# facebookresearch/fast3r

Measured on AMD Instinct MI355X. Metric: views/sec (512^2, ViT-L) single forward pass at N=320, higher is better.
Workload: dtype fp16

## Files before the change

fast3r_amd/csrc/f3r_capi.hip:

```cpp
#include <stdarg.h>
#include <stdio.h>

#include "f3r_common.h"

namespace {
thread_local char g_err[512] = "";
}

void f3r_set_error(const char* fmt, ...) {
  va_list ap;
  va_start(ap, fmt);
  vsnprintf(g_err, sizeof(g_err), fmt, ap);
  va_end(ap);
}

int f3r_check_launch(const char* what) {
  hipError_t e = hipGetLastError();
  if (e != hipSuccess) {
    f3r_set_error("%s: launch failed: %s", what, hipGetErrorString(e));
    return F3R_ERR_LAUNCH;
  }
  return F3R_OK;
}

extern "C" int f3r_version(void) { return 380;  }

extern "C" int f3r_wall_clock_khz(void) {
  int dev = 0, khz = 0;
  if (hipGetDevice(&dev) != hipSuccess || hipDeviceGetAttribute(&khz, hipDeviceAttributeWallClockRate, dev) != hipSuccess) {
    (void)hipGetLastError();
    return 0;
  }
  return khz;
}

extern "C" const char* f3r_last_error_string(void) { return g_err; }

extern "C" size_t f3r_sizeof(int what) {
  switch (what) {
    case 0: return sizeof(f3r_gemm_args);
// ... 26 lines not shown
```

fast3r_amd/csrc/f3r_gemm.hip:

```cpp
#include <stdlib.h>

#include "f3r_common.h"
#include "f3r_gemm_epi.h"

namespace {

constexpr int BM = 128, BN = 128, BK = 64, NT = 256;
constexpr int TILE_ELEMS = 128 * 64;
constexpr int GEMM_LDS_BYTES = 2 * 2 * TILE_ELEMS * 2;

__device__ __forceinline__ int swz(int row, int chunk) { return row * 64 + ((chunk ^ ((row >> 1) & 7)) << 3); }

struct ConvRow {
  int b, oy, ox;
  bool ok;
};

template <class T, int A_MODE, int EPI, int GLDS>
__global__ __launch_bounds__(NT, 2) void gemm_kernel(const f3r_gemm_args p) {
  extern __shared__ __attribute__((aligned(16))) uint16_t smem[];
  uint16_t* As = smem;
  uint16_t* Ws = smem + 2 * TILE_ELEMS;

  const int tid = threadIdx.x;
// ... 284 lines not shown
    }
    if (!f3r_gemm_asm_f8_eligible(a, &why)) {
      f3r_set_error("f3r_gemm: split W2F8 (fp8 low plane) but the launch is not eligible for the hand-scheduled kernel: %s", why);
      return F3R_ERR_UNSUPPORTED;
    }
    return f3r_gemm_asm_f8_launch(a, (hipStream_t)stream);
  }
  F3R_REQUIRE(a.epi == F3R_EPI_GENERIC || (!a.out_f8 && !a.out_relu_f8 && !a.fin_w), "f3r_gemm: out_f8 / out_relu_f8 / fin_w need the generic epilogue (epi %d)", a.epi);
  const int planes = a.split ? 2 : 1;
  F3R_REQUIRE(a.Kpad > 0 && a.Kpad % (64 * planes) == 0, "f3r_gemm: Kpad %d must be a positive multiple of %d", a.Kpad, 64 * planes);
  const int Kpad1 = a.Kpad / planes;
  F3R_REQUIRE((a.split != F3R_SPLIT_X3 && a.split != F3R_SPLIT_X3F8) || (a.A_lo && al16(a.A_lo) && !a.a_relu), "f3r_gemm: X3 / X3F8 split needs A_lo (16-byte aligned) and no a_relu");
  if (a.split == F3R_SPLIT_X3F8)
    F3R_REQUIRE(a.a_mode == F3R_A_CONV3X3 && a.dtype == F3R_F16 && a.conv_C % 128 == 0 && a.w_scale && (((uintptr_t)a.w_scale) & 3) == 0,
                "f3r_gemm: X3F8 needs a 3x3 convolution with conv_C %% 128 == 0 (got %d), fp16 planes and w_scale", a.conv_C);
  F3R_REQUIRE((a.kernel_sel >= 0 && a.kernel_sel <= 7) || a.kernel_sel == 9 || a.kernel_sel >= 16, "f3r_gemm: bad kernel_sel %d", a.kernel_sel);
  F3R_REQUIRE(a.N % 4 == 0, "f3r_gemm: N %d must be a multiple of 4", a.N);
  F3R_REQUIRE(al16(a.A) && al16(a.W), "f3r_gemm: A/W must be 16-byte aligned");
  F3R_REQUIRE(a.dtype == F3R_F16 || a.dtype == F3R_BF16, "f3r_gemm: bad dtype %d", a.dtype);
  if (a.a_mode == F3R_A_PLAIN) {
    F3R_REQUIRE(a.K > 0 && a.K % 8 == 0 && a.K <= Kpad1, "f3r_gemm: K %d must be a multiple of 8 and <= Kpad", a.K);
    F3R_REQUIRE(a.lda % 8 == 0 && a.lda >= a.K, "f3r_gemm: lda %lld must be a multiple of 8 and >= K", (long long)a.lda);
  } else if (a.a_mode == F3R_A_CONV3X3) {
    F3R_REQUIRE(a.conv_C > 0 && a.conv_C % 8 == 0, "f3r_gemm: conv_C %d must be a multiple of 8", a.conv_C);
    F3R_REQUIRE(Kpad1 == 9 * ((a.conv_C + 63) / 64) * 64, "f3r_gemm: conv Kpad %d != 9*roundup(C,64) per plane", a.Kpad);
    F3R_REQUIRE(a.epi == F3R_EPI_GENERIC, "f3r_gemm: conv3x3 supports only the generic epilogue");
    F3R_REQUIRE(a.conv_stride == 1 || a.conv_stride == 2, "f3r_gemm: conv stride %d", a.conv_stride);
    F3R_REQUIRE(a.conv_OH == (a.conv_H + 2 - 3) / a.conv_stride + 1 && a.conv_OW == (a.conv_W + 2 - 3) / a.conv_stride + 1,
                "f3r_gemm: conv output dims inconsistent");
    F3R_REQUIRE(a.conv_OH > 0 && a.conv_OW > 0 && a.M % ((int64_t)a.conv_OH * a.conv_OW) == 0, "f3r_gemm: conv M not a multiple of OH*OW");
  } else {
// ... 69 lines not shown
```

fast3r_amd/csrc/f3r_gemm256.hip:

```cpp
#include "f3r_gemm256_impl.h"

int f3r_gemm256_run_bf16(const f3r_gemm_args& a, hipStream_t stream, int stagger);
int f3r_gemm256_run_conv_f8_fin(const f3r_gemm_args& a, hipStream_t stream);

bool f3r_gemm256_eligible(const f3r_gemm_args& a) {
  if (a.N % 128 != 0) return false;
  if (a.epi == F3R_EPI_QKV) {
    const int Dq = a.qkv_dq ? a.qkv_dq : a.N / 3;
    if (Dq % 256 != 0 || ((a.N - Dq) / 2) % 256 != 0) return false;
  }
  const int Kpad1 = a.split ? a.Kpad / 2 : a.Kpad;
  if (Kpad1 % 64 != 0) return false;
  if (a.a_mode == F3R_A_PLAIN) {
    if (a.K != Kpad1) return false;
    if ((int64_t)256 * a.lda * 2 >= (1ll << 32)) return false;
  } else {
    if (a.a_relu || a.conv_C % 64 != 0) return false;
    if (a.M / ((int64_t)a.conv_OH * a.conv_OW) * a.conv_H * a.conv_W * a.conv_C * 2 >= (1ll << 32)) return false;
    if (a.split == F3R_SPLIT_X3F8 && (a.conv_C % 128 != 0 || a.dtype != F3R_F16)) return false;
  }
  if (a.split == F3R_SPLIT_X3F8 && a.a_mode != F3R_A_CONV3X3) return false;
  if (a.fin_w && (a.a_mode != F3R_A_CONV3X3 || a.N != 128 || a.epi != F3R_EPI_GENERIC)) return false;
  if ((int64_t)256 * a.Kpad * 2 >= (1ll << 32)) return false;
  const int add = gemm_additive_pattern(a);
  if (add == F3R_ADD_UNSUPPORTED || (add != F3R_ADD_NONE && a.act != F3R_ACT_NONE)) return false;
  if (add != F3R_ADD_NONE && a.epi != F3R_EPI_GENERIC) return false;
  if (a.a_mode == F3R_A_CONV3X3 ? (add == F3R_ADD_RES_F32 || add == F3R_ADD_ROWADD) : add == F3R_ADD_RES_LP) return false;
  return true;
}

bool f3r_gemm256_preferred(const f3r_gemm_args& a) { return score_256(a, tile_halves(a)) >= score_128(a); }

int f3r_gemm256_launch(const f3r_gemm_args& a, hipStream_t stream, int stagger) {
  const int64_t tiles = ((a.M + BM - 1) / BM) * ((a.N + 127) / 128);
// ... 6 lines not shown
```

fast3r_amd/csrc/f3r_gemm256_f8.hip:

```cpp
#include <cstdlib>

#include "f3r_gemm256_impl.h"

int f3r_gemm256_run_conv_f8_fin(const f3r_gemm_args& a, hipStream_t stream) {
  const bool f8 = a.split == F3R_SPLIT_X3F8;
  const int add = gemm_additive_pattern(a);
  if (a.fin_w) {
#ifdef F3R_CONV_ABLATIONS
    if (f8) {
      static const char* ab = getenv("F3R_CONV_ABLATE");
      switch (ab ? atoi(ab) : 0) {
#define F3R_ABL(n) case n: return launch256<F16, F3R_A_CONV3X3, F3R_EPI_GENERIC, 1, F3R_ADD_NONE, 1, true, true, false, n>(a, stream);
        F3R_ABL(1) F3R_ABL(1024) F3R_ABL(2048) F3R_ABL(2) F3R_ABL(4) F3R_ABL(3) F3R_ABL(7)
#undef F3R_ABL
      }
    }
#endif
    if (a.dtype == F3R_BF16) return launch256<BF16, F3R_A_CONV3X3, F3R_EPI_GENERIC, 1, F3R_ADD_NONE, 1, false, true>(a, stream);
    if (f8 && a.kernel_sel == 5) return launch256<F16, F3R_A_CONV3X3, F3R_EPI_GENERIC, 1, F3R_ADD_NONE, 1, true, true, true>(a, stream);
    return f8 ? launch256<F16, F3R_A_CONV3X3, F3R_EPI_GENERIC, 1, F3R_ADD_NONE, 1, true, true>(a, stream)
              : launch256<F16, F3R_A_CONV3X3, F3R_EPI_GENERIC, 1, F3R_ADD_NONE, 1, false, true>(a, stream);
  }
  const int nh = tile_halves(a);
  if (add == F3R_ADD_RES_LP)
    return nh == 2 ? launch256<F16, F3R_A_CONV3X3, F3R_EPI_GENERIC, 1, F3R_ADD_RES_LP, 2, true>(a, stream)
                   : launch256<F16, F3R_A_CONV3X3, F3R_EPI_GENERIC, 1, F3R_ADD_RES_LP, 1, true>(a, stream);
  return nh == 2 ? launch256<F16, F3R_A_CONV3X3, F3R_EPI_GENERIC, 1, F3R_ADD_NONE, 2, true>(a, stream)
                 : launch256<F16, F3R_A_CONV3X3, F3R_EPI_GENERIC, 1, F3R_ADD_NONE, 1, true>(a, stream);
}
```

fast3r_amd/csrc/f3r_gemm256_impl.h:

```cpp
#pragma once
#include <atomic>

#include "f3r_common.h"
#include "f3r_gemm_epi.h"


namespace {

constexpr int BM = 256, BK = 64, NT = 512;
constexpr int HT = 128 * 64;
template <int NH> struct TileCfg {
  static constexpr int BN = 128 * NH;
  static constexpr int BUF = (2 + NH) * HT;
  static constexpr int NBUF = NH == 2 ? 2 : 3;
  static constexpr int TAB_ENTRIES = 512;
  static constexpr int LDS_BYTES = NBUF * BUF * 2 + TAB_ENTRIES * 16;
};

inline int f3r_num_cus() {
  constexpr int MAXD = 64;
  static std::atomic<int> cache[MAXD];
  int dev = 0;
  if (hipGetDevice(&dev) != hipSuccess) dev = 0;
  if (dev >= 0 && dev < MAXD) {
    const int c = cache[dev].load(std::memory_order_relaxed);
    if (c) return c;
  }
  int cu = 0;
  if (hipDeviceGetAttribute(&cu, hipDeviceAttributeMultiprocessorCount, dev) != hipSuccess || cu < 8) cu = 256;
  const int n = cu / 8 * 8;
  if (dev >= 0 && dev < MAXD) cache[dev].store(n, std::memory_order_relaxed);
  return n;
}

typedef __attribute__((address_space(3))) void* lds_ptr_t;
typedef const __attribute__((address_space(1))) void* glb_ptr_t;

template <int V>
struct IC {
  static constexpr int value = V;
};

#define F3R_VMCNT(n) __builtin_amdgcn_s_waitcnt(0x0F70 | (n))
#define F3R_LGKMCNT0() __builtin_amdgcn_s_waitcnt(0xC07F)

template <class T, int A_MODE, int EPI, bool SWAP, int STAGGER, int ADDSRC, int NH = 2, int LAB = 0, bool F8 = false, bool FIN = false, bool MERGED = false>
__device__ __forceinline__ void gemm256_body(const f3r_gemm_args& p, uint16_t* smem, const int64_t m0_tile, const int n0_tile, const bool first = true,
                                             const bool has_next = false, const int64_t m0_next = 0, const int n0_next = 0) {
  constexpr int BUF = TileCfg<NH>::BUF;
  int64_t m0 = m0_tile;
  int n0 = n0_tile;
  const int tid = threadIdx.x;
  const int lane = tid & 63;
  const int wid = __builtin_amdgcn_readfirstlane(tid >> 6);
  const int wm = wid >> 2, wn = wid & 3;
  const int fr = lane & 15, fg = lane >> 4;
  constexpr bool PAIRED = EPI != F3R_EPI_QKV && (ADDSRC == F3R_ADD_NONE || ADDSRC == F3R_ADD_RES_LP);
  static_assert(!(PAIRED && SWAP), "swapped roles exist only in the QKV role");
  auto w_key = [](int r) { return PAIRED ? (((r >> 1) & 1) | (((r >> 3) & 3) << 1)) : ((r >> 1) & 7); };
  uint64_t stamp[5] = {0, 0, 0, 0, 0};
  if (LAB & 128) stamp[0] = __builtin_amdgcn_s_memtime();
  if ((LAB & (256 | 512)) && blockIdx.x < 256) {
    const int PH = (LAB & 512) ? 4 : 2;
// ... 2 lines not shown
    for (int i = 0; i < n; ++i) __builtin_amdgcn_s_sleep(15);
  }

  const int nseg = p.split == F3R_SPLIT_NONE ? 1 : (p.split == F3R_SPLIT_W2 ? 2 : 3);
  const int Kpad1 = p.split == F3R_SPLIT_NONE ? p.Kpad : p.Kpad / 2;
  const int nk1 = Kpad1 / BK;
  const int nk8 = nk1 / 2;
  const int nk = F8 ? nk1 + 2 * nk8 : nseg * nk1;
  const int ctiles = A_MODE == F3R_A_CONV3X3 ? p.conv_C / 64 : 1;
  const int ctiles8 = A_MODE == F3R_A_CONV3X3 ? p.conv_C / 128 : 1;
  static_assert(!F8 || (A_MODE == F3R_A_CONV3X3 && !SWAP), "fp8 correction segments: convolutions only");
  static_assert(!FIN || (NH == 1 && EPI == F3R_EPI_GENERIC && ADDSRC == 0 && !SWAP), "fused head tail: 256 x 128 tiles, no additive terms");

  uint32_t a_off[2][2], w_off[2][2];
  uint32_t a_msk[2][2];
  const char* const Ab = (const char*)p.A;
  const char* const Alo = (const char*)p.A_lo;
  const uint32_t a_bytes = A_MODE == F3R_A_CONV3X3 ? (uint32_t)(p.M / ((int64_t)p.conv_OH * p.conv_OW) * p.conv_H * p.conv_W * p.conv_C * 2) : 0u;
  const char* Wb = nullptr;
  uint32_t wsc[NH][2];
  auto setup_tile = [&](int64_t tm0, int tn0) {
  m0 = tm0;
  n0 = tn0;
  Wb = (const char*)p.W + (int64_t)n0 * p.Kpad * 2;
  if constexpr (F8) {
#pragma unroll
    for (int h = 0; h < NH; ++h)
#pragma unroll
      for (int nf = 0; nf < 2; ++nf) {
        int n = n0 + h * 128 + (wid & 3) * 32 + (PAIRED ? (fr >> 2) * 8 + (fr & 3) + nf * 4 : fr + nf * 16);
        if (n >= p.N) n = p.N - 1;
        wsc[h][nf] = p.w_scale[n];
      }
  }
#pragma unroll
  for (int h = 0; h < 2; ++h)
#pragma unroll
    for (int i = 0; i < 2; ++i) {
      const int r = (wid * 2 + i) * 8 + (lane >> 3);
      const int lc = (lane & 7) ^ ((r >> 1) & 7);
      int n = n0 + (h < NH ? h : 0) * 128 + r;
      if (n >= p.N) n = p.N - 1;
      w_off[h][i] = (uint32_t)(((int64_t)(n - n0) * p.Kpad + ((lane & 7) ^ w_key(r)) * 8) * 2);
      int64_t m = m0 + h * 128 + r;
      if (A_MODE == F3R_A_PLAIN) {
        if (m >= p.M) m = p.M - 1;
        a_off[h][i] = (uint32_t)(((m - m0) * p.lda + lc * 8) * 2);
        a_msk[h][i] = 0;
      } else {
        const bool ok = m < p.M;
        const int64_t per_img = (int64_t)p.conv_OH * p.conv_OW;
        const int64_t mm = ok ? m : 0;
        const int b = (int)(mm / per_img);
        const int rem = (int)(mm % per_img);
        const int oy = rem / p.conv_OW, ox = rem - oy * p.conv_OW;
        const int cy = oy * p.conv_stride, cx = ox * p.conv_stride;
        a_off[h][i] = (uint32_t)(((((int64_t)b * p.conv_H + cy) * p.conv_W + cx) * p.conv_C + lc * 8) * 2);
        uint32_t msk = 0;
#pragma unroll
        for (int tap = 0; tap < 9; ++tap) {
          const int iy = cy + tap / 3 - 1, ix = cx + tap % 3 - 1;
          if (!(ok && iy >= 0 && iy < p.conv_H && ix >= 0 && ix < p.conv_W)) msk |= 1u << tap;
        }
        a_msk[h][i] = msk;
      }
    }
  };
  setup_tile(m0_tile, n0_tile);

  constexpr bool TAB = A_MODE == F3R_A_CONV3X3;
  const int pix = TAB ? p.conv_C * 2 : 0;
  uint32_t* const tab = (uint32_t*)(smem + TileCfg<NH>::NBUF * BUF);
  if (TAB && first) {
    for (int t = tid; t < nk; t += NT) {
      int delta, meta, wso;
      if (!F8 || t < nk1) {
        const int seg = F8 ? 0 : t / nk1, kk = t - seg * nk1, tapn = kk / ctiles, ct = kk - tapn * ctiles;
        delta = ((tapn / 3 - 1) * p.conv_W + (tapn % 3 - 1)) * pix + ct * 128;
        meta = tapn | ((!F8 && seg == 2) ? 16 : 0);
        wso = ((seg == 1 ? Kpad1 : 0) + kk * BK) * 2;
      } else {
        const int u = t - nk1, s8 = u / nk8, kk = u - s8 * nk8, tapn = kk / ctiles8, ct = kk - tapn * ctiles8;
        delta = ((tapn / 3 - 1) * p.conv_W + (tapn % 3 - 1)) * pix + (s8 == 1 ? p.conv_C : 0) + ct * 128;
        meta = tapn | 16;
        wso = (s8 + 2) * Kpad1 + kk * 128;
      }
      *(u32x4*)(tab + t * 4) = u32x4{(uint32_t)delta, (uint32_t)meta, (uint32_t)wso, 0u};
    }
    __syncthreads();
  }
  u32x4 ea = {0u, 0u, 0u, 0u}, ew = ea;
  int a_seg = 0, a_kk = 0, a_t = 0;
  int w_seg = 0, w_kk = 0, w_t = 0;
  auto fetch = [&]() {
    if constexpr (TAB) {
      ea = *(const u32x4*)(tab + a_t * 4);
      ew = *(const u32x4*)(tab + w_t * 4);
    }
  };
  bool dry = false;
  auto a_advance = [&]() {
    if (a_t + 1 < nk) {
      ++a_t;
      if constexpr (!TAB) {
        ++a_kk;
        if (a_kk == nk1) { a_kk = 0; ++a_seg; }
      }
    }
  };
  auto w_advance = [&]() {
    if (w_t + 1 < nk) {
      ++w_t;
      if constexpr (!TAB) {
        ++w_kk;
        if (w_kk == nk1) { w_kk = 0; ++w_seg; }
      }
    }
  };
  bool in_loop = false;
  auto issue_a = [&](int h, int buf) {
    if (dry) return;
    if ((LAB & (1 | 2048)) && in_loop) return;
    const char* plane = (!TAB && a_seg == 2) ? Alo : Ab;
    uint16_t* dst = smem + buf * BUF + h * HT + wid * 2 * 8 * 64;
    if (A_MODE == F3R_A_PLAIN) {
      const char* base = plane + (m0 * p.lda + (int64_t)a_kk * BK) * 2;
      if (LAB & 32) {
        const __amdgpu_buffer_rsrc_t rs = __builtin_amdgcn_make_buffer_rsrc((void*)(plane + m0 * p.lda * 2), 0, 0x7fffffff, 0x00020000);
#pragma unroll
        for (int i = 0; i < 2; ++i)
          __builtin_amdgcn_raw_ptr_buffer_load_lds(rs, (lds_ptr_t)(dst + i * 8 * 64), 16, (int)a_off[h][i], a_kk * BK * 2, 0, 0);
        return;
      }
#pragma unroll
// ... 4 lines not shown
      const int meta = __builtin_amdgcn_readfirstlane((int)ea[1]);
      const int a_tap = meta & 15;
      const char* pl = (meta & 16) ? Alo : Ab;
      const __amdgpu_buffer_rsrc_t rs = __builtin_amdgcn_make_buffer_rsrc((void*)pl, 0, a_bytes, 0x00020000);
#pragma unroll
      for (int i = 0; i < 2; ++i) {
        const int32_t inv = ((int32_t)(a_msk[h][i] << (31 - a_tap))) >> 31;
        const uint32_t vo = (a_off[h][i] + (uint32_t)a_delta) | (uint32_t)inv;
        __builtin_amdgcn_raw_ptr_buffer_load_lds(rs, (lds_ptr_t)(dst + i * 8 * 64), 16, (int)vo, 0, 0, 0);
      }
    }
  };
  auto issue_w = [&](int h, int buf) {
    if (dry) return;
    if ((LAB & (1 | 1024)) && in_loop) return;
    uint16_t* dst = smem + buf * BUF + (2 + h) * HT + wid * 2 * 8 * 64;
    if constexpr (TAB) {
      const int w_soff = __builtin_amdgcn_readfirstlane((int)ew[2]);
      const __amdgpu_buffer_rsrc_t rs = __builtin_amdgcn_make_buffer_rsrc((void*)Wb, 0, 0x7fffffff, 0x00020000);
#pragma unroll
      for (int i = 0; i < 2; ++i)
        __builtin_amdgcn_raw_ptr_buffer_load_lds(rs, (lds_ptr_t)(dst + i * 8 * 64), 16, (int)w_off[h][i], w_soff, 0, 0);
      return;
    }
    const char* base = Wb + ((int64_t)(w_seg == 1 ? Kpad1 : 0) + (int64_t)w_kk * BK) * 2;
    if (LAB & 32) {
      const __amdgpu_buffer_rsrc_t rs = __builtin_amdgcn_make_buffer_rsrc((void*)Wb, 0, 0x7fffffff, 0x00020000);
#pragma unroll
      for (int i = 0; i < 2; ++i)
        __builtin_amdgcn_raw_ptr_buffer_load_lds(rs, (lds_ptr_t)(dst + i * 8 * 64), 16, (int)w_off[h][i], ((w_seg == 1 ? Kpad1 : 0) + w_kk * BK) * 2, 0, 0);
      return;
    }
#pragma unroll
    for (int i = 0; i < 2; ++i)
      __builtin_amdgcn_global_load_lds((glb_ptr_t)(base + w_off[h][i]), (lds_ptr_t)(dst + i * 8 * 64), 16, 0, 0);
  };

  const int sw = (fr >> 1) & 7;
  const int w_row = wn * 32 + (PAIRED ? (fr >> 2) * 8 + (fr & 3) : fr);
  int a_rd[2], w_rd[2];
#pragma unroll
  for (int ks = 0; ks < 2; ++ks) {
    a_rd[ks] = (wm * 64 + fr) * 64 + (((ks * 4 + fg) ^ sw) << 3);
    w_rd[ks] = w_row * 64 + (((ks * 4 + fg) ^ w_key(w_row)) << 3);
  }

  float4v acc[16 * NH];
  typename T::vec8 fa0[2][4], fa1[2][4], fw[2][2];
  typedef uint32_t u32x8 __attribute__((ext_vector_type(8)));
  typedef int i32x8 __attribute__((ext_vector_type(8)));
  u32x8 ga0[4], ga1[4], gw[2];

  auto read_a = [&](auto e8, auto which, int buf, int mh) {
    if ((LAB & 2) && in_loop) return;
    if constexpr (decltype(e8)::value) {
      auto& g = decltype(which)::value ? ga1 : ga0;
#pragma unroll
      for (int mf = 0; mf < 4; ++mf) {
        const u32x4 c0 = *(const u32x4*)(smem + buf * BUF + mh * HT + a_rd[0] + mf * 16 * 64);
        const u32x4 c1 = *(const u32x4*)(smem + buf * BUF + mh * HT + a_rd[1] + mf * 16 * 64);
        g[mf] = __builtin_shufflevector(c0, c1, 0, 1, 2, 3, 4, 5, 6, 7);
      }
    } else {
      auto& f = decltype(which)::value ? fa1 : fa0;
#pragma unroll
      for (int ks = 0; ks < 2; ++ks)
#pragma unroll
        for (int mf = 0; mf < 4; ++mf)
          f[ks][mf] = as_vec8<T>(*(const u32x4*)(smem + buf * BUF + mh * HT + a_rd[ks] + mf * 16 * 64));
    }
  };
  auto read_w = [&](auto e8, int buf, int nh) {
    if ((LAB & 2) && in_loop) return;
    if constexpr (decltype(e8)::value) {
#pragma unroll
      for (int nf = 0; nf < 2; ++nf) {
        const u32x4 c0 = *(const u32x4*)(smem + buf * BUF + (2 + nh) * HT + w_rd[0] + nf * (PAIRED ? 4 : 16) * 64);
        const u32x4 c1 = *(const u32x4*)(smem + buf * BUF + (2 + nh) * HT + w_rd[1] + nf * (PAIRED ? 4 : 16) * 64);
        gw[nf] = __builtin_shufflevector(c0, c1, 0, 1, 2, 3, 4, 5, 6, 7);
      }
    } else {
#pragma unroll
      for (int ks = 0; ks < 2; ++ks)
#pragma unroll
        for (int nf = 0; nf < 2; ++nf)
          fw[ks][nf] = as_vec8<T>(*(const u32x4*)(smem + buf * BUF + (2 + nh) * HT + w_rd[ks] + nf * (PAIRED ? 4 : 16) * 64));
    }
  };
  auto mma = [&](auto e8, auto which, int mh, int nh, int sa_shift, int sb) {
    if (LAB & 4) return;
    if constexpr (decltype(e8)::value) {
      auto& g = decltype(which)::value ? ga1 : ga0;
#pragma unroll
      for (int nf = 0; nf < 2; ++nf) {
        const int sa = (int)((wsc[nh < NH ? nh : 0][nf] >> sa_shift) & 0xffu);
#pragma unroll
        for (int mf = 0; mf < 4; ++mf) {
          const int NF = nh * 2 + nf, MF = mh * 4 + mf;
          acc[NF * 8 + MF] = __builtin_amdgcn_mfma_scale_f32_16x16x128_f8f6f4(__builtin_bit_cast(i32x8, gw[nf]), __builtin_bit_cast(i32x8, g[mf]),
                                                                              acc[NF * 8 + MF], 0, 0, 0, sa, 0, sb);
        }
// ... 56 lines not shown
    constexpr int B = decltype(bufc)::value;
    constexpr int B2 = (B + 2) % 3;
    fetch();
    read_w(e8, B, 0);
    if (!(LAB & 64)) __builtin_amdgcn_sched_barrier(0);
    read_a(e8, IC<0>{}, B, 0);
    issue_a(0, B2);
    issue_w(0, B2);
    w_advance();
    if (!(LAB & 8)) F3R_VMCNT(10);
    F3R_PHASE_MMA(0, 0, 0)
    read_a(e8, IC<1>{}, B, 1);
    issue_a(1, B2);
    a_advance();
    if (!(LAB & 8)) F3R_VMCNT(8);
    F3R_PHASE_MMA(1, 1, 0)
  };
#define F3R_MMA2_OPEN()                                  \
  __builtin_amdgcn_sched_barrier(0);                     \
  __builtin_amdgcn_s_barrier();                          \
  F3R_LGKMCNT0();                                        \
  __builtin_amdgcn_sched_barrier(0);                     \
  __builtin_amdgcn_s_setprio(1);
#define F3R_MMA2_ISSUE()                                 \
  __builtin_amdgcn_s_setprio(0);                         \
  __builtin_amdgcn_sched_barrier(0);
#define F3R_MMA2_CLOSE()                                 \
  __builtin_amdgcn_sched_barrier(0);                     \
  __builtin_amdgcn_s_barrier();
  auto tileM = [&](auto bufc, auto e8, int sa_shift, int sb) {
// ... 43 lines not shown
    mma(e8, IC<1>{}, 1, 0, sa_shift, sb);
    F3R_MMA2_ISSUE()
    F3R_MMA2_CLOSE()
  };
#undef F3R_MMA2_OPEN
#undef F3R_MMA2_ISSUE
#undef F3R_MMA2_CLOSE
#undef F3R_PHASE_MMA

  typedef GemmFragLayout<2 * NH, 8, 2, 4, PAIRED> Frag;
  const int64_t m_base = m0_tile + wm * 64;
  const int n_base = n0_tile + wn * 32;
  auto opening_loads = [&]() {
    a_seg = a_kk = a_t = 0;
    w_seg = w_kk = w_t = 0;
    if constexpr (NH == 2) {
      if (!dry) fetch();
      issue_a(0, 0);
      issue_w(0, 0);
      issue_a(1, 0);
      a_advance();
      issue_w(1, 0);
      w_advance();
      if (!dry) fetch();
      issue_a(0, 1);
      issue_w(0, 1);
      if constexpr (MERGED) {
        issue_a(1, 1);
        a_advance();
      }
    } else {
// ... 6 lines not shown
      if (!dry) fetch();
      issue_a(0, 1);
      issue_w(0, 1);
      w_advance();
      issue_a(1, 1);
      a_advance();
    }
  };
  dry = !first;
  opening_loads();
  dry = false;
  gemm_acc_init_additive<T, Frag, ADDSRC, SWAP>(p, acc, m_base, n_base, lane);
  if (first && MERGED) {
    if constexpr (NH == 2) F3R_VMCNT(8);
    else F3R_VMCNT(6);
  } else if (first) {
    F3R_VMCNT(8);
  } else {
    F3R_VMCNT(0);
  }
  __builtin_amdgcn_s_barrier();
  if (STAGGER && wm == 1) __builtin_amdgcn_s_barrier();
  if (LAB & 128) stamp[1] = __builtin_amdgcn_s_memtime();

  typedef IC<0> E16;
  typedef IC<1> E8;
  auto T2 = [&](auto bufc, auto e8, int sa_shift, int sb) {
    if constexpr (MERGED) tileM(bufc, e8, sa_shift, sb);
    else tile(bufc, e8, sa_shift, sb);
  };
  auto T1 = [&](auto bufc, auto e8, int sa_shift, int sb) {
    if constexpr (MERGED) tile1M(bufc, e8, sa_shift, sb);
    else tile1(bufc, e8, sa_shift, sb);
  };
  const int nk16 = F8 ? nk1 : nk;
  if constexpr (NH == 2) {
    if (LAB) {
      tile(IC<0>{}, E16{}, 0, 0);
      if (nk > 1) tile(IC<1>{}, E16{}, 0, 0);
      in_loop = true;
    }
    for (int t = LAB ? 2 : 0; t < nk16; t += 2) {
      T2(IC<0>{}, E16{}, 0, 0);
      if (t + 1 < nk16) T2(IC<1>{}, E16{}, 0, 0);
    }
    if constexpr (F8) {
      for (int t = 0; t < nk1; t += 2) {
        T2(IC<0>{}, E8{}, t >= nk8 ? 8 : 0, t >= nk8 ? 115 : 127);
        T2(IC<1>{}, E8{}, t + 1 >= nk8 ? 8 : 0, t + 1 >= nk8 ? 115 : 127);
      }
    }
// ... 10 lines not shown
        T1(IC<1>{}, E8{}, t + 1 >= nk8 ? 8 : 0, t + 1 >= nk8 ? 115 : 127);
        T1(IC<2>{}, E8{}, t + 2 >= nk8 ? 8 : 0, t + 2 >= nk8 ? 115 : 127);
      }
    }
  }
  F3R_VMCNT(0);
  if (STAGGER && wm == 0) __builtin_amdgcn_s_barrier();
  if (LAB & 128) stamp[2] = __builtin_amdgcn_s_memtime();
  if (has_next) {
    setup_tile(m0_next, n0_next);
    opening_loads();
  }

  if constexpr (FIN) {
    __builtin_amdgcn_s_barrier();
    gemm_epilogue_fin<T, Frag>(p, acc, m0_tile, wm, wn, lane, tid, (float*)(smem + 2 * BUF));
  } else if (SWAP) gemm_epilogue_vt<T, Frag, false>(p, acc, m_base, n_base, lane);
  else gemm_epilogue_default<T, EPI, Frag, false>(p, acc, m_base, n_base, lane);
  if (LAB & 128) {
    __builtin_amdgcn_sched_barrier(0);
    stamp[3] = __builtin_amdgcn_s_memtime();
    F3R_VMCNT(0);
    stamp[4] = __builtin_amdgcn_s_memtime();
    if (tid == 0) {
      uint64_t* d = (uint64_t*)p.rope_cos + (int64_t)blockIdx.x * 5;
      for (int i = 0; i < 5; ++i) d[i] = stamp[i];
    }
  }
}

template <class T, int A_MODE, int EPI, int STAGGER, int ADDSRC, int NH, bool F8 = false, bool FIN = false, bool MERGED = false, int LAB = 0>
__global__ __launch_bounds__(NT, 1) void gemm256_kernel(const f3r_gemm_args p) {
  extern __shared__ __attribute__((aligned(16))) uint16_t smem[];
  constexpr int BN = TileCfg<NH>::BN;
  const int n_tiles_n = (p.N + BN - 1) / BN;
  const int64_t n_tiles_m = (p.M + BM - 1) / BM;
  const int64_t n_wg = n_tiles_m * n_tiles_n;
  auto tile_of = [&](int64_t wg, int64_t& m0, int& n0) {
    {
      const int64_t q = n_wg / 8, r = n_wg % 8;
      const int64_t xcd = wg % 8, idx = wg / 8;
      wg = (xcd < r ? xcd * (q + 1) : r * (q + 1) + (xcd - r) * q) + idx;
    }
    constexpr int GM = 8;
    const int64_t per_group = (int64_t)GM * n_tiles_n;
    const int64_t grp = wg / per_group;
// ... 7 lines not shown
  };
  int64_t m0, m0n = 0;
  int n0, n0n = 0;
  bool first = true;
  for (int64_t v = blockIdx.x; v < n_wg; v += gridDim.x) {
    tile_of(v, m0, n0);
    const bool has_next = v + gridDim.x < n_wg;
    if (has_next) tile_of(v + gridDim.x, m0n, n0n);
    bool done = false;
    if constexpr (EPI == F3R_EPI_QKV) {
      if (n0 >= (p.qkv_dq ? p.qkv_dq + (p.N - p.qkv_dq) / 2 : 2 * (p.N / 3))) {
        gemm256_body<T, A_MODE, EPI, true, STAGGER, F3R_ADD_NONE, NH>(p, smem, m0, n0, first, has_next, m0n, n0n);
        done = true;
      }
    }
    if (!done) gemm256_body<T, A_MODE, EPI, false, STAGGER, ADDSRC, NH, LAB, F8, FIN, MERGED>(p, smem, m0, n0, first, has_next, m0n, n0n);
    first = false;
  }
}

template <class T, int A_MODE, int EPI, int STAGGER, int ADDSRC, int NH, bool F8 = false, bool FIN = false, bool MERGED = false, int LAB = 0>
int launch256(const f3r_gemm_args& a, hipStream_t stream) {
  static bool attr_set = false;
  auto kern = gemm256_kernel<T, A_MODE, EPI, STAGGER, ADDSRC, NH, F8, FIN, MERGED, LAB>;
  constexpr int LDS_BYTES = TileCfg<NH>::LDS_BYTES, BN = TileCfg<NH>::BN;
  if (!attr_set) {
    (void)hipFuncSetAttribute((const void*)kern, hipFuncAttributeMaxDynamicSharedMemorySize, LDS_BYTES);
    attr_set = true;
  }
  const int64_t tiles = ((a.M + BM - 1) / BM) * ((a.N + BN - 1) / BN);
  const int64_t grid = (a.kernel_sel == 5 || tiles <= f3r_num_cus()) ? tiles : f3r_num_cus();
  hipLaunchKernelGGL(kern, dim3((unsigned)grid), dim3(NT), LDS_BYTES, stream, a);
  return f3r_check_launch("f3r_gemm(256)");
}

inline float tile_score(int64_t tiles, int slots, float eff) {
  if (tiles <= 0) return 0.f;
  const int64_t rounds = (tiles + slots - 1) / slots;
  return eff * (float)tiles / (float)(rounds * slots);
}
inline float score_256(const f3r_gemm_args& a, int nh) {
  return tile_score(((a.M + 255) / 256) * ((a.N + 128 * nh - 1) / (128 * nh)), 256, nh == 2 ? 1.0f : 0.82f);
}
inline float score_128(const f3r_gemm_args& a) { return tile_score(((a.M + 127) / 128) * ((a.N + 127) / 128), 512, 0.72f); }

inline int tile_halves(const f3r_gemm_args& a) {
  if (a.epi == F3R_EPI_QKV) return 2;
  if (a.N % 256 != 0 || a.kernel_sel == 4) return 1;
  if (a.kernel_sel == 2 || a.kernel_sel == 3 || a.kernel_sel == 5) return 2;
  return score_256(a, 1) > score_256(a, 2) ? 1 : 2;
}

template <class T>
int dispatch256(const f3r_gemm_args& a, hipStream_t stream, int stagger) {
#define F3R_L256H(AM, EP, AD, NHV) (stagger ? launch256<T, AM, EP, 1, AD, NHV>(a, stream) : launch256<T, AM, EP, 0, AD, NHV>(a, stream))
#define F3R_L256(AM, EP, AD) (nh == 2 ? F3R_L256H(AM, EP, AD, 2) : F3R_L256H(AM, EP, AD, 1))
  const int add = gemm_additive_pattern(a);
  const int nh = tile_halves(a);
  if (a.a_mode == F3R_A_CONV3X3) return add == F3R_ADD_RES_LP ? F3R_L256(F3R_A_CONV3X3, F3R_EPI_GENERIC, F3R_ADD_RES_LP) : F3R_L256(F3R_A_CONV3X3, F3R_EPI_GENERIC, F3R_ADD_NONE);
  switch (a.epi) {
    case F3R_EPI_GENERIC:
      return add == F3R_ADD_RES_F32 ? F3R_L256(F3R_A_PLAIN, F3R_EPI_GENERIC, F3R_ADD_RES_F32)
           : add == F3R_ADD_ROWADD ? F3R_L256(F3R_A_PLAIN, F3R_EPI_GENERIC, F3R_ADD_ROWADD) : F3R_L256(F3R_A_PLAIN, F3R_EPI_GENERIC, F3R_ADD_NONE);
    case F3R_EPI_QKV: return F3R_L256H(F3R_A_PLAIN, F3R_EPI_QKV, F3R_ADD_NONE, 2);
    default: return F3R_L256(F3R_A_PLAIN, F3R_EPI_CONVT, F3R_ADD_NONE);
  }
#undef F3R_L256
#undef F3R_L256H
}

#ifdef F3R_GEMM_LAB
template <class T, int LAB>
__global__ __launch_bounds__(NT, 1) void gemm256_lab_kernel(const f3r_gemm_args p) {
  extern __shared__ __attribute__((aligned(16))) uint16_t smem[];
// ... 18 lines not shown
```

Before: 35.73.

## Stage 3x3 conv input as row strips reused across horizontal taps

Adds a strip-staging mode to the 256-row implicit-GEMM conv kernel for stride-1 3x3 convolutions whose output width divides or is a multiple of 256. Each A strip (tile rows plus halo) is loaded once into LDS and read at three horizontal offsets, so the three dx taps share one global load instead of issuing three. This reduces A-operand global/LDS traffic for the DPT head convolutions. In exchange it adds a new LDS layout, reworked k-tables, hand-scheduled stile pipelines with new waitcnt values, more template instantiations, and risk of scheduling or correctness errors. Kernel_sel 8 is kept as an opt-out that uses the old per-tap staging.

```diff
diff --git a/fast3r_amd/csrc/f3r_capi.hip b/fast3r_amd/csrc/f3r_capi.hip
--- a/fast3r_amd/csrc/f3r_capi.hip
+++ b/fast3r_amd/csrc/f3r_capi.hip
@@ -23,7 +23,7 @@
   return F3R_OK;
 }
 
-extern "C" int f3r_version(void) { return 380;  }
+extern "C" int f3r_version(void) { return 390;  }
 
 extern "C" int f3r_wall_clock_khz(void) {
   int dev = 0, khz = 0;
diff --git a/fast3r_amd/csrc/f3r_gemm.hip b/fast3r_amd/csrc/f3r_gemm.hip
--- a/fast3r_amd/csrc/f3r_gemm.hip
+++ b/fast3r_amd/csrc/f3r_gemm.hip
@@ -322,7 +322,8 @@
   if (a.split == F3R_SPLIT_X3F8)
     F3R_REQUIRE(a.a_mode == F3R_A_CONV3X3 && a.dtype == F3R_F16 && a.conv_C % 128 == 0 && a.w_scale && (((uintptr_t)a.w_scale) & 3) == 0,
                 "f3r_gemm: X3F8 needs a 3x3 convolution with conv_C %% 128 == 0 (got %d), fp16 planes and w_scale", a.conv_C);
-  F3R_REQUIRE((a.kernel_sel >= 0 && a.kernel_sel <= 7) || a.kernel_sel == 9 || a.kernel_sel >= 16, "f3r_gemm: bad kernel_sel %d", a.kernel_sel);
+  F3R_REQUIRE((a.kernel_sel >= 0 && a.kernel_sel <= 9) || a.kernel_sel >= 16, "f3r_gemm: bad kernel_sel %d", a.kernel_sel);
+  F3R_REQUIRE(a.kernel_sel != 8 || a.a_mode == F3R_A_CONV3X3, "f3r_gemm: kernel_sel 8 (per-tap staging) is a choice of the 3x3 convolutions");
   F3R_REQUIRE(a.N % 4 == 0, "f3r_gemm: N %d must be a multiple of 4", a.N);
   F3R_REQUIRE(al16(a.A) && al16(a.W), "f3r_gemm: A/W must be 16-byte aligned");
   F3R_REQUIRE(a.dtype == F3R_F16 || a.dtype == F3R_BF16, "f3r_gemm: bad dtype %d", a.dtype);
diff --git a/fast3r_amd/csrc/f3r_gemm256.hip b/fast3r_amd/csrc/f3r_gemm256.hip
--- a/fast3r_amd/csrc/f3r_gemm256.hip
+++ b/fast3r_amd/csrc/f3r_gemm256.hip
@@ -18,6 +18,8 @@
     if (a.a_relu || a.conv_C % 64 != 0) return false;
     if (a.M / ((int64_t)a.conv_OH * a.conv_OW) * a.conv_H * a.conv_W * a.conv_C * 2 >= (1ll << 32)) return false;
     if (a.split == F3R_SPLIT_X3F8 && (a.conv_C % 128 != 0 || a.dtype != F3R_F16)) return false;
+    const int nk1 = Kpad1 / 64;
+    if ((a.split == F3R_SPLIT_X3 ? 3 * nk1 : a.split == F3R_SPLIT_NONE ? nk1 : 2 * nk1) > F3R_TAB_ENTRIES) return false;
   }
   if (a.split == F3R_SPLIT_X3F8 && a.a_mode != F3R_A_CONV3X3) return false;
   if (a.fin_w && (a.a_mode != F3R_A_CONV3X3 || a.N != 128 || a.epi != F3R_EPI_GENERIC)) return false;
diff --git a/fast3r_amd/csrc/f3r_gemm256_f8.hip b/fast3r_amd/csrc/f3r_gemm256_f8.hip
--- a/fast3r_amd/csrc/f3r_gemm256_f8.hip
+++ b/fast3r_amd/csrc/f3r_gemm256_f8.hip
@@ -16,15 +16,21 @@
       }
     }
 #endif
-    if (a.dtype == F3R_BF16) return launch256<BF16, F3R_A_CONV3X3, F3R_EPI_GENERIC, 1, F3R_ADD_NONE, 1, false, true>(a, stream);
-    if (f8 && a.kernel_sel == 5) return launch256<F16, F3R_A_CONV3X3, F3R_EPI_GENERIC, 1, F3R_ADD_NONE, 1, true, true, true>(a, stream);
-    return f8 ? launch256<F16, F3R_A_CONV3X3, F3R_EPI_GENERIC, 1, F3R_ADD_NONE, 1, true, true>(a, stream)
-              : launch256<F16, F3R_A_CONV3X3, F3R_EPI_GENERIC, 1, F3R_ADD_NONE, 1, false, true>(a, stream);
+    const int strip = f3r_conv_strip_form(a);
+#define F3R_FIN(TT, F8V, MG, ST) launch256<TT, F3R_A_CONV3X3, F3R_EPI_GENERIC, 1, F3R_ADD_NONE, 1, F8V, true, MG, 0, ST>(a, stream)
+    if (a.dtype == F3R_BF16) return strip == 1 ? F3R_FIN(BF16, false, false, 1) : strip == 2 ? F3R_FIN(BF16, false, false, 2) : F3R_FIN(BF16, false, false, 0);
+    if (f8 && a.kernel_sel == 5) return F3R_FIN(F16, true, true, 0);
+    if (strip == 1) return f8 ? F3R_FIN(F16, true, false, 1) : F3R_FIN(F16, false, false, 1);
+    if (strip == 2) return f8 ? F3R_FIN(F16, true, false, 2) : F3R_FIN(F16, false, false, 2);
+    return f8 ? F3R_FIN(F16, true, false, 0) : F3R_FIN(F16, false, false, 0);
+#undef F3R_FIN
   }
   const int nh = tile_halves(a);
-  if (add == F3R_ADD_RES_LP)
-    return nh == 2 ? launch256<F16, F3R_A_CONV3X3, F3R_EPI_GENERIC, 1, F3R_ADD_RES_LP, 2, true>(a, stream)
-                   : launch256<F16, F3R_A_CONV3X3, F3R_EPI_GENERIC, 1, F3R_ADD_RES_LP, 1, true>(a, stream);
-  return nh == 2 ? launch256<F16, F3R_A_CONV3X3, F3R_EPI_GENERIC, 1, F3R_ADD_NONE, 2, true>(a, stream)
-                 : launch256<F16, F3R_A_CONV3X3, F3R_EPI_GENERIC, 1, F3R_ADD_NONE, 1, true>(a, stream);
+  const int strip = f3r_conv_strip_form(a);
+#define F3R_F8(AD, NHV, ST) launch256<F16, F3R_A_CONV3X3, F3R_EPI_GENERIC, 1, AD, NHV, true, false, false, 0, ST>(a, stream)
+#define F3R_F8N(AD, ST) (nh == 2 ? F3R_F8(AD, 2, ST) : F3R_F8(AD, 1, ST))
+  if (add == F3R_ADD_RES_LP) return strip == 1 ? F3R_F8N(F3R_ADD_RES_LP, 1) : strip == 2 ? F3R_F8N(F3R_ADD_RES_LP, 2) : F3R_F8N(F3R_ADD_RES_LP, 0);
+  return strip == 1 ? F3R_F8N(F3R_ADD_NONE, 1) : strip == 2 ? F3R_F8N(F3R_ADD_NONE, 2) : F3R_F8N(F3R_ADD_NONE, 0);
+#undef F3R_F8N
+#undef F3R_F8
 }
diff --git a/fast3r_amd/csrc/f3r_gemm256_impl.h b/fast3r_amd/csrc/f3r_gemm256_impl.h
--- a/fast3r_amd/csrc/f3r_gemm256_impl.h
+++ b/fast3r_amd/csrc/f3r_gemm256_impl.h
@@ -9,12 +9,18 @@
 
 constexpr int BM = 256, BK = 64, NT = 512;
 constexpr int HT = 128 * 64;
-template <int NH> struct TileCfg {
+constexpr int STRIP_ROWS = 288;
+constexpr int STRIP_BYTES = STRIP_ROWS * 128;
+constexpr int F3R_TAB_ENTRIES = 512;
+template <int NH, bool STRIP = false> struct TileCfg {
   static constexpr int BN = 128 * NH;
   static constexpr int BUF = (2 + NH) * HT;
   static constexpr int NBUF = NH == 2 ? 2 : 3;
-  static constexpr int TAB_ENTRIES = 512;
-  static constexpr int LDS_BYTES = NBUF * BUF * 2 + TAB_ENTRIES * 16;
+  static constexpr int TAB_ENTRIES = F3R_TAB_ENTRIES;
+  static constexpr int WRING = STRIP ? 2 * STRIP_BYTES / 2 : 0;
+  static constexpr int TAB_OFF = STRIP ? WRING + NBUF * NH * HT : NBUF * BUF;
+  static constexpr int DUMP_OFF = TAB_OFF + TAB_ENTRIES * 8;
+  static constexpr int LDS_BYTES = TAB_OFF * 2 + TAB_ENTRIES * 16 + (STRIP ? 1024 : 0);
 };
 
 inline int f3r_num_cus() {
@@ -44,9 +50,11 @@
 #define F3R_VMCNT(n) __builtin_amdgcn_s_waitcnt(0x0F70 | (n))
 #define F3R_LGKMCNT0() __builtin_amdgcn_s_waitcnt(0xC07F)
 
-template <class T, int A_MODE, int EPI, bool SWAP, int STAGGER, int ADDSRC, int NH = 2, int LAB = 0, bool F8 = false, bool FIN = false, bool MERGED = false>
+template <class T, int A_MODE, int EPI, bool SWAP, int STAGGER, int ADDSRC, int NH = 2, int LAB = 0, bool F8 = false, bool FIN = false, bool MERGED = false,
+          int STRIP = 0>
 __device__ __forceinline__ void gemm256_body(const f3r_gemm_args& p, uint16_t* smem, const int64_t m0_tile, const int n0_tile, const bool first = true,
                                              const bool has_next = false, const int64_t m0_next = 0, const int n0_next = 0) {
+  static_assert(STRIP == 0 || (A_MODE == F3R_A_CONV3X3 && !SWAP && !MERGED && LAB == 0), "strip staging: product convolutions only");
   constexpr int BUF = TileCfg<NH>::BUF;
   int64_t m0 = m0_tile;
   int n0 = n0_tile;
@@ -79,6 +87,10 @@
 
   uint32_t a_off[2][2], w_off[2][2];
   uint32_t a_msk[2][2];
+  uint32_t s_off[5] = {0u, 0u, 0u, 0u, 0u};
+  uint32_t s_msk = 0;
+  const int s_wp = STRIP ? (p.conv_W < 256 ? p.conv_W : 256) : 1;
+  const int s_lw = 31 - __builtin_clz(s_wp);
   const char* const Ab = (const char*)p.A;
   const char* const Alo = (const char*)p.A_lo;
   const uint32_t a_bytes = A_MODE == F3R_A_CONV3X3 ? (uint32_t)(p.M / ((int64_t)p.conv_OH * p.conv_OW) * p.conv_H * p.conv_W * p.conv_C * 2) : 0u;
@@ -108,7 +120,8 @@
       if (n >= p.N) n = p.N - 1;
       w_off[h][i] = (uint32_t)(((int64_t)(n - n0) * p.Kpad + ((lane & 7) ^ w_key(r)) * 8) * 2);
       int64_t m = m0 + h * 128 + r;
-      if (A_MODE == F3R_A_PLAIN) {
+      if constexpr (STRIP != 0) {
+      } else if (A_MODE == F3R_A_PLAIN) {
         if (m >= p.M) m = p.M - 1;
         a_off[h][i] = (uint32_t)(((m - m0) * p.lda + lc * 8) * 2);
         a_msk[h][i] = 0;
@@ -130,16 +143,52 @@
         a_msk[h][i] = msk;
       }
     }
+  if constexpr (STRIP != 0) {
+    s_msk = 0;
+#pragma unroll
+    for (int i = 0; i < 5; ++i) {
+      const int r = (wid + 8 * i) * 8 + (lane >> 3);
+      const int g = r / (s_wp + 2);
+      const int j = r - g * (s_wp + 2) - 1;
+      const int64_t ms = m0 + (int64_t)g * s_wp;
+      const bool ok = r < 256 + 2 * (256 >> s_lw) && ms < p.M;
+      const int64_t per_img = (int64_t)p.conv_H * p.conv_W;
+      const int64_t mm = ok ? ms : 0;
+      const int b = (int)(mm / per_img);
+      const int rem = (int)(mm % per_img);
+      const int oy = rem / p.conv_W, ix = rem - oy * p.conv_W + j;
+      const int lc = (lane & 7) ^ (((r - 2 * g) >> 1) & 7);
+      s_off[i] = (uint32_t)(((((int64_t)b * p.conv_H + oy) * p.conv_W + ix) * p.conv_C + lc * 8) * 2);
+      const bool in_x = ok && ix >= 0 && ix < p.conv_W;
+      uint32_t msk = 0;
+#pragma unroll
+      for (int dy = 0; dy < 3; ++dy)
+        if (!(in_x && oy + dy - 1 >= 0 && oy + dy - 1 < p.conv_H)) msk |= 1u << dy;
+      s_msk |= msk << (3 * i);
+    }
+  }
   };
   setup_tile(m0_tile, n0_tile);
 
   constexpr bool TAB = A_MODE == F3R_A_CONV3X3;
   const int pix = TAB ? p.conv_C * 2 : 0;
-  uint32_t* const tab = (uint32_t*)(smem + TileCfg<NH>::NBUF * BUF);
+  uint32_t* const tab = (uint32_t*)(smem + TileCfg<NH, (STRIP != 0)>::TAB_OFF);
   if (TAB && first) {
     for (int t = tid; t < nk; t += NT) {
       int delta, meta, wso;
-      if (!F8 || t < nk1) {
+      if constexpr (STRIP != 0) {
+        if (!F8 || t < nk1) {
+          const int seg = F8 ? 0 : t / nk1, kk = t - seg * nk1, s = kk / 3, dx = kk - s * 3, dy = s / ctiles, ct = s - dy * ctiles;
+          delta = (dy - 1) * p.conv_W * pix + ct * 128;
+          meta = dy | ((!F8 && seg == 2) ? 16 : 0);
+          wso = ((seg == 1 ? Kpad1 : 0) + ((dy * 3 + dx) * ctiles + ct) * BK) * 2;
+        } else {
+          const int u = t - nk1, s8 = u / nk8, kk = u - s8 * nk8, s = kk / 3, dx = kk - s * 3, dy = s / ctiles8, ct = s - dy * ctiles8;
+          delta = (dy - 1) * p.conv_W * pix + (s8 == 1 ? p.conv_C : 0) + ct * 128;
+          meta = dy | 16;
+          wso = (s8 + 2) * Kpad1 + ((dy * 3 + dx) * ctiles8 + ct) * 128;
+        }
+      } else if (!F8 || t < nk1) {
         const int seg = F8 ? 0 : t / nk1, kk = t - seg * nk1, tapn = kk / ctiles, ct = kk - tapn * ctiles;
         delta = ((tapn / 3 - 1) * p.conv_W + (tapn % 3 - 1)) * pix + ct * 128;
         meta = tapn | ((!F8 && seg == 2) ? 16 : 0);
@@ -165,6 +214,10 @@
   };
   bool dry = false;
   auto a_advance = [&]() {
+    if constexpr (STRIP != 0) {
+      if (a_t + 3 < nk) a_t += 3;
+      return;
+    }
     if (a_t + 1 < nk) {
       ++a_t;
       if constexpr (!TAB) {
@@ -183,6 +236,23 @@
     }
   };
   bool in_loop = false;
+  auto w_slot = [](int buf, int h) { return STRIP ? TileCfg<NH, (STRIP != 0)>::WRING + (buf * NH + h) * HT : buf * BUF + (2 + h) * HT; };
+  auto issue_s = [&](auto i0c, auto nc, auto sbc) {
+    if (dry) return;
+    constexpr int I0 = decltype(i0c)::value, N = decltype(nc)::value, SB = decltype(sbc)::value;
+    const int a_delta = __builtin_amdgcn_readfirstlane((int)ea[0]);
+    const int meta = __builtin_amdgcn_readfirstlane((int)ea[1]);
+    const int dy = meta & 15;
+    const char* pl = (meta & 16) ? Alo : Ab;
+    const __amdgpu_buffer_rsrc_t rs = __builtin_amdgcn_make_buffer_rsrc((void*)pl, 0, a_bytes, 0x00020000);
+#pragma unroll
+    for (int i = I0; i < I0 + N; ++i) {
+      const int32_t inv = ((int32_t)(s_msk << (31 - 3 * i - dy))) >> 31;
+      const uint32_t vo = (s_off[i] + (uint32_t)a_delta) | (uint32_t)inv;
+      uint16_t* dst = (i == 4 && wid >= 4) ? smem + TileCfg<NH, (STRIP != 0)>::DUMP_OFF : smem + SB * (STRIP_BYTES / 2) + (wid + 8 * i) * 8 * 64;
+      __builtin_amdgcn_raw_ptr_buffer_load_lds(rs, (lds_ptr_t)dst, 16, (int)vo, 0, 0, 0);
+    }
+  };
   auto issue_a = [&](int h, int buf) {
     if (dry) return;
     if ((LAB & (1 | 2048)) && in_loop) return;
@@ -217,7 +287,7 @@
   auto issue_w = [&](int h, int buf) {
     if (dry) return;
     if ((LAB & (1 | 1024)) && in_loop) return;
-    uint16_t* dst = smem + buf * BUF + (2 + h) * HT + wid * 2 * 8 * 64;
+    uint16_t* dst = smem + w_slot(buf, h) + wid * 2 * 8 * 64;
     if constexpr (TAB) {
       const int w_soff = __builtin_amdgcn_readfirstlane((int)ew[2]);
       const __amdgpu_buffer_rsrc_t rs = __builtin_amdgcn_make_buffer_rsrc((void*)Wb, 0, 0x7fffffff, 0x00020000);
@@ -246,6 +316,20 @@
   for (int ks = 0; ks < 2; ++ks) {
     a_rd[ks] = (wm * 64 + fr) * 64 + (((ks * 4 + fg) ^ sw) << 3);
     w_rd[ks] = w_row * 64 + (((ks * 4 + fg) ^ w_key(w_row)) << 3);
+  }
+
+  int s_rd[3][2] = {{0, 0}, {0, 0}, {0, 0}};
+  int s_goff[2][4] = {{0, 0, 0, 0}, {0, 0, 0, 0}};
+  if constexpr (STRIP != 0) {
+#pragma unroll
+    for (int k = 0; k < 3; ++k)
+#pragma unroll
+      for (int ks = 0; ks < 2; ++ks)
+        s_rd[k][ks] = (wm * 64 + fr + k + (STRIP == 1 ? 2 * ((wm * 64) >> s_lw) : 0)) * 64 + (((ks * 4 + fg) ^ (((fr + k) >> 1) & 7)) << 3);
+#pragma unroll
+    for (int mh = 0; mh < 2; ++mh)
+#pragma unroll
+      for (int mf = 0; mf < 4; ++mf) s_goff[mh][mf] = 2 * ((STRIP == 1 ? mh * 128 : mh * 128 + wm * 64 + mf * 16) >> s_lw) * 64;
   }
 
   float4v acc[16 * NH];
@@ -273,13 +357,44 @@
           f[ks][mf] = as_vec8<T>(*(const u32x4*)(smem + buf * BUF + mh * HT + a_rd[ks] + mf * 16 * 64));
     }
   };
+  auto read_sa = [&](auto e8, auto which, auto kc, auto sbc, int mh) {
+    constexpr int K = decltype(kc)::value, SB = decltype(sbc)::value;
+    if constexpr (decltype(e8)::value) {
+      auto& g = decltype(which)::value ? ga1 : ga0;
+#pragma unroll
+      for (int mf = 0; mf < 4; ++mf) {
+        int go = 0;
+        if (STRIP == 2 || mh) {
+          go = s_goff[mh][mf];
+          asm volatile("" : "+s"(go));
+        }
+        const uint16_t* b = smem + SB * (STRIP_BYTES / 2) + (mh * 128 + mf * 16) * 64 + go;
+        const u32x4 c0 = *(const u32x4*)(b + s_rd[K][0]);
+        const u32x4 c1 = *(const u32x4*)(b + s_rd[K][1]);
+        g[mf] = __builtin_shufflevector(c0, c1, 0, 1, 2, 3, 4, 5, 6, 7);
+      }
+    } else {
+      auto& f = decltype(which)::value ? fa1 : fa0;
+#pragma unroll
+      for (int ks = 0; ks < 2; ++ks)
+#pragma unroll
+        for (int mf = 0; mf < 4; ++mf) {
+          int go = 0;
+          if (STRIP == 2 || mh) {
+            go = s_goff[mh][mf];
+            asm volatile("" : "+s"(go));
+          }
+          f[ks][mf] = as_vec8<T>(*(const u32x4*)(smem + SB * (STRIP_BYTES / 2) + (mh * 128 + mf * 16) * 64 + go + s_rd[K][ks]));
+        }
+    }
+  };
   auto read_w = [&](auto e8, int buf, int nh) {
     if ((LAB & 2) && in_loop) return;
     if constexpr (decltype(e8)::value) {
 #pragma unroll
       for (int nf = 0; nf < 2; ++nf) {
-        const u32x4 c0 = *(const u32x4*)(smem + buf * BUF + (2 + nh) * HT + w_rd[0] + nf * (PAIRED ? 4 : 16) * 64);
-        const u32x4 c1 = *(const u32x4*)(smem + buf * BUF + (2 + nh) * HT + w_rd[1] + nf * (PAIRED ? 4 : 16) * 64);
+        const u32x4 c0 = *(const u32x4*)(smem + w_slot(buf, nh) + w_rd[0] + nf * (PAIRED ? 4 : 16) * 64);
+        const u32x4 c1 = *(const u32x4*)(smem + w_slot(buf, nh) + w_rd[1] + nf * (PAIRED ? 4 : 16) * 64);
         gw[nf] = __builtin_shufflevector(c0, c1, 0, 1, 2, 3, 4, 5, 6, 7);
       }
     } else {
@@ -287,7 +402,7 @@
       for (int ks = 0; ks < 2; ++ks)
 #pragma unroll
         for (int nf = 0; nf < 2; ++nf)
-          fw[ks][nf] = as_vec8<T>(*(const u32x4*)(smem + buf * BUF + (2 + nh) * HT + w_rd[ks] + nf * (PAIRED ? 4 : 16) * 64));
+          fw[ks][nf] = as_vec8<T>(*(const u32x4*)(smem + w_slot(buf, nh) + w_rd[ks] + nf * (PAIRED ? 4 : 16) * 64));
     }
   };
   auto mma = [&](auto e8, auto which, int mh, int nh, int sa_shift, int sb) {
@@ -374,6 +489,52 @@
     issue_a(1, B2);
     a_advance();
     if (!(LAB & 8)) F3R_VMCNT(8);
+    F3R_PHASE_MMA(1, 1, 0)
+  };
+  auto stile = [&](auto kc, auto bufc, auto sbc, auto e8, int sa_shift, int sb) {
+    constexpr int K = decltype(kc)::value, B = decltype(bufc)::value, SB = decltype(sbc)::value;
+    fetch();
+    read_w(e8, B, 0);
+    __builtin_amdgcn_sched_barrier(0);
+    read_sa(e8, IC<0>{}, kc, sbc, 0);
+    if constexpr (K == 0) issue_s(IC<0>{}, IC<2>{}, IC<SB ^ 1>{});
+    if constexpr (K == 1) {
+      issue_s(IC<4>{}, IC<1>{}, IC<SB ^ 1>{});
+      a_advance();
+    }
+    F3R_PHASE_MMA(0, 0, 0)
+    fetch();
+    read_sa(e8, IC<1>{}, kc, sbc, 1);
+    issue_w(1, B ^ 1);
+    w_advance();
+    F3R_VMCNT(K == 0 ? 6 : K == 1 ? 7 : 4);
+    F3R_PHASE_MMA(1, 1, 0)
+    fetch();
+    read_w(e8, B, 1);
+    if constexpr (K == 0) issue_s(IC<2>{}, IC<2>{}, IC<SB ^ 1>{});
+    F3R_PHASE_MMA(1, 1, 1)
+    fetch();
+    issue_w(0, B);
+    F3R_VMCNT(K == 0 ? 8 : K == 1 ? 5 : 4);
+    F3R_PHASE_MMA(0, 0, 1)
+  };
+  auto stile1 = [&](auto kc, auto sbc, auto e8, int sa_shift, int sb) {
+    constexpr int K = decltype(kc)::value, SB = decltype(sbc)::value;
+    constexpr int B = K, B2 = (K + 2) % 3;
+    fetch();
+    read_w(e8, B, 0);
+    __builtin_amdgcn_sched_barrier(0);
+    read_sa(e8, IC<0>{}, kc, sbc, 0);
+    if constexpr (K == 1) {
+      issue_s(IC<3>{}, IC<2>{}, IC<SB ^ 1>{});
+      a_advance();
+    }
+    issue_w(0, B2);
+    w_advance();
+    F3R_PHASE_MMA(0, 0, 0)
+    read_sa(e8, IC<1>{}, kc, sbc, 1);
+    if constexpr (K == 0) issue_s(IC<0>{}, IC<3>{}, IC<SB ^ 1>{});
+    F3R_VMCNT(K == 0 ? 5 : K == 1 ? 7 : 2);
     F3R_PHASE_MMA(1, 1, 0)
   };
 #define F3R_MMA2_OPEN()                                  \
@@ -447,7 +608,17 @@
   auto opening_loads = [&]() {
     a_seg = a_kk = a_t = 0;
     w_seg = w_kk = w_t = 0;
-    if constexpr (NH == 2) {
+    if constexpr (STRIP != 0) {
+      if (!dry) fetch();
+      issue_s(IC<0>{}, IC<5>{}, IC<0>{});
+      a_advance();
+      issue_w(0, 0);
+      if constexpr (NH == 2) issue_w(1, 0);
+      w_advance();
+      if (!dry) fetch();
+      issue_w(0, 1);
+      if constexpr (NH == 1) w_advance();
+    } else if constexpr (NH == 2) {
       if (!dry) fetch();
       issue_a(0, 0);
       issue_w(0, 0);
@@ -484,6 +655,9 @@
   if (first && MERGED) {
     if constexpr (NH == 2) F3R_VMCNT(8);
     else F3R_VMCNT(6);
+  } else if (first && STRIP) {
+    if constexpr (NH == 2) F3R_VMCNT(4);
+    else F3R_VMCNT(2);
   } else if (first) {
     F3R_VMCNT(8);
   } else {
@@ -504,7 +678,32 @@
     else tile1(bufc, e8, sa_shift, sb);
   };
   const int nk16 = F8 ? nk1 : nk;
-  if constexpr (NH == 2) {
+  if constexpr (STRIP != 0) {
+    auto strip3 = [&](auto sbc, auto e8, int sa_shift, int sb) {
+      constexpr int SB = decltype(sbc)::value;
+      if constexpr (NH == 2) {
+        stile(IC<0>{}, IC<SB>{}, sbc, e8, sa_shift, sb);
+        stile(IC<1>{}, IC<SB ^ 1>{}, sbc, e8, sa_shift, sb);
+        stile(IC<2>{}, IC<SB>{}, sbc, e8, sa_shift, sb);
+      } else {
+        stile1(IC<0>{}, sbc, e8, sa_shift, sb);
+        stile1(IC<1>{}, sbc, e8, sa_shift, sb);
+        stile1(IC<2>{}, sbc, e8, sa_shift, sb);
+      }
+    };
+    const int ns16 = nk16 / 3;
+    for (int s = 0; s < ns16; s += 2) {
+      strip3(IC<0>{}, E16{}, 0, 0);
+      if (s + 1 < ns16) strip3(IC<1>{}, E16{}, 0, 0);
+    }
+    if constexpr (F8) {
+      const int ns8 = nk8 / 3;
+      for (int s = 0; s < 2 * ns8; s += 2) {
+        strip3(IC<0>{}, E8{}, s >= ns8 ? 8 : 0, s >= ns8 ? 115 : 127);
+        strip3(IC<1>{}, E8{}, s + 1 >= ns8 ? 8 : 0, s + 1 >= ns8 ? 115 : 127);
+      }
+    }
+  } else if constexpr (NH == 2) {
     if (LAB) {
       tile(IC<0>{}, E16{}, 0, 0);
       if (nk > 1) tile(IC<1>{}, E16{}, 0, 0);
@@ -545,7 +744,7 @@
 
   if constexpr (FIN) {
     __builtin_amdgcn_s_barrier();
-    gemm_epilogue_fin<T, Frag>(p, acc, m0_tile, wm, wn, lane, tid, (float*)(smem + 2 * BUF));
+    gemm_epilogue_fin<T, Frag>(p, acc, m0_tile, wm, wn, lane, tid, (float*)(smem + (STRIP ? STRIP_BYTES / 2 : 2 * BUF)));
   } else if (SWAP) gemm_epilogue_vt<T, Frag, false>(p, acc, m_base, n_base, lane);
   else gemm_epilogue_default<T, EPI, Frag, false>(p, acc, m_base, n_base, lane);
   if (LAB & 128) {
@@ -560,7 +759,7 @@
   }
 }
 
-template <class T, int A_MODE, int EPI, int STAGGER, int ADDSRC, int NH, bool F8 = false, bool FIN = false, bool MERGED = false, int LAB = 0>
+template <class T, int A_MODE, int EPI, int STAGGER, int ADDSRC, int NH, bool F8 = false, bool FIN = false, bool MERGED = false, int LAB = 0, int STRIP = 0>
 __global__ __launch_bounds__(NT, 1) void gemm256_kernel(const f3r_gemm_args p) {
   extern __shared__ __attribute__((aligned(16))) uint16_t smem[];
   constexpr int BN = TileCfg<NH>::BN;
@@ -598,16 +797,16 @@
         done = true;
       }
     }
-    if (!done) gemm256_body<T, A_MODE, EPI, false, STAGGER, ADDSRC, NH, LAB, F8, FIN, MERGED>(p, smem, m0, n0, first, has_next, m0n, n0n);
+    if (!done) gemm256_body<T, A_MODE, EPI, false, STAGGER, ADDSRC, NH, LAB, F8, FIN, MERGED, STRIP>(p, smem, m0, n0, first, has_next, m0n, n0n);
     first = false;
   }
 }
 
-template <class T, int A_MODE, int EPI, int STAGGER, int ADDSRC, int NH, bool F8 = false, bool FIN = false, bool MERGED = false, int LAB = 0>
+template <class T, int A_MODE, int EPI, int STAGGER, int ADDSRC, int NH, bool F8 = false, bool FIN = false, bool MERGED = false, int LAB = 0, int STRIP = 0>
 int launch256(const f3r_gemm_args& a, hipStream_t stream) {
   static bool attr_set = false;
-  auto kern = gemm256_kernel<T, A_MODE, EPI, STAGGER, ADDSRC, NH, F8, FIN, MERGED, LAB>;
-  constexpr int LDS_BYTES = TileCfg<NH>::LDS_BYTES, BN = TileCfg<NH>::BN;
+  auto kern = gemm256_kernel<T, A_MODE, EPI, STAGGER, ADDSRC, NH, F8, FIN, MERGED, LAB, STRIP>;
+  constexpr int LDS_BYTES = TileCfg<NH, (STRIP != 0)>::LDS_BYTES, BN = TileCfg<NH>::BN;
   if (!attr_set) {
     (void)hipFuncSetAttribute((const void*)kern, hipFuncAttributeMaxDynamicSharedMemorySize, LDS_BYTES);
     attr_set = true;
@@ -627,6 +826,13 @@
   return tile_score(((a.M + 255) / 256) * ((a.N + 128 * nh - 1) / (128 * nh)), 256, nh == 2 ? 1.0f : 0.82f);
 }
 inline float score_128(const f3r_gemm_args& a) { return tile_score(((a.M + 127) / 128) * ((a.N + 127) / 128), 512, 0.72f); }
+
+inline bool f3r_conv_strip_eligible(const f3r_gemm_args& a) {
+  if (a.a_mode != F3R_A_CONV3X3 || a.conv_stride != 1 || a.kernel_sel == 8) return false;
+  const int W = a.conv_OW;
+  return W >= 16 && (256 % W == 0 || W % 256 == 0);
+}
+inline int f3r_conv_strip_form(const f3r_gemm_args& a) { return !f3r_conv_strip_eligible(a) ? 0 : a.conv_OW >= 64 ? 1 : 2; }
 
 inline int tile_halves(const f3r_gemm_args& a) {
   if (a.epi == F3R_EPI_QKV) return 2;
@@ -641,7 +847,18 @@
 #define F3R_L256(AM, EP, AD) (nh == 2 ? F3R_L256H(AM, EP, AD, 2) : F3R_L256H(AM, EP, AD, 1))
   const int add = gemm_additive_pattern(a);
   const int nh = tile_halves(a);
-  if (a.a_mode == F3R_A_CONV3X3) return add == F3R_ADD_RES_LP ? F3R_L256(F3R_A_CONV3X3, F3R_EPI_GENERIC, F3R_ADD_RES_LP) : F3R_L256(F3R_A_CONV3X3, F3R_EPI_GENERIC, F3R_ADD_NONE);
+  if (a.a_mode == F3R_A_CONV3X3) {
+#define F3R_L256S(AD, NHV, ST) (stagger ? launch256<T, F3R_A_CONV3X3, F3R_EPI_GENERIC, 1, AD, NHV, false, false, false, 0, ST>(a, stream) \
+                                        : launch256<T, F3R_A_CONV3X3, F3R_EPI_GENERIC, 0, AD, NHV, false, false, false, 0, ST>(a, stream))
+#define F3R_L256C(AD, ST) (nh == 2 ? F3R_L256S(AD, 2, ST) : F3R_L256S(AD, 1, ST))
+    switch (f3r_conv_strip_form(a)) {
+      case 1: return add == F3R_ADD_RES_LP ? F3R_L256C(F3R_ADD_RES_LP, 1) : F3R_L256C(F3R_ADD_NONE, 1);
+      case 2: return add == F3R_ADD_RES_LP ? F3R_L256C(F3R_ADD_RES_LP, 2) : F3R_L256C(F3R_ADD_NONE, 2);
+      default: return add == F3R_ADD_RES_LP ? F3R_L256C(F3R_ADD_RES_LP, 0) : F3R_L256C(F3R_ADD_NONE, 0);
+    }
+#undef F3R_L256C
+#undef F3R_L256S
+  }
   switch (a.epi) {
     case F3R_EPI_GENERIC:
       return add == F3R_ADD_RES_F32 ? F3R_L256(F3R_A_PLAIN, F3R_EPI_GENERIC, F3R_ADD_RES_F32)
```

Measured after the change: 35.37. Within noise of the previous version (-1.0%).
